# src-d/kmcuda

Hardware: AMD Instinct MI355X
Metric: point-assignments/sec per Lloyd iter (8Mx256@1024) (higher is better)
Workload: dtype f32

## Files before the change

include/kmcuda_amd.h:

```cpp
#ifndef KMCUDA_AMD_H
#define KMCUDA_AMD_H

#include <stddef.h>
#include <stdint.h>

#ifdef __cplusplus
extern "C" {
#endif

typedef struct kmamd_engine kmamd_engine;

int kmamd_engine_create(kmamd_engine **out, int device, uint32_t n_rows, uint32_t features,
                        uint32_t clusters, int metric, int fp16x2, void *hip_stream);
void kmamd_engine_destroy(kmamd_engine *e);
void *kmamd_engine_stream(kmamd_engine *e);
int kmamd_engine_sync(kmamd_engine *e);

int kmamd_lloyd_assign(kmamd_engine *e, const float *samples, const float *centroids,
                       uint32_t *assignments, uint32_t *assignments_prev);
int kmamd_lloyd_assign_exact(kmamd_engine *e, const float *samples, const float *centroids,
                             uint32_t *assignments, uint32_t *assignments_prev);

int kmamd_set_filter(kmamd_engine *e, int mode);

int kmamd_set_half_rows(kmamd_engine *e, const void *rows16);

int kmamd_set_row_cache(kmamd_engine *e, int on);

int kmamd_counters_read(kmamd_engine *e, uint32_t *host_out4);
int kmamd_counters_reset(kmamd_engine *e, int which );
int kmamd_yy_hint_stats(kmamd_engine *e, uint32_t *host_out6);

int kmamd_move_deltas(kmamd_engine *e, const float *samples, const uint32_t *assignments_prev,
                      const uint32_t *assignments, double *delta, int32_t *dcount);
int kmamd_apply_delta(kmamd_engine *e, const double *delta, const int32_t *dcount,
                      float *centroids, uint32_t *ccounts);
size_t kmamd_reduce_len(kmamd_engine *e);
int kmamd_reduce_fill(kmamd_engine *e, const float *samples, const uint32_t *assignments_prev,
                      const uint32_t *assignments, double *buf);
int kmamd_reduce_apply(kmamd_engine *e, const double *buf, float *centroids, uint32_t *ccounts);
int kmamd_reduce_apply_stop(kmamd_engine *e, const double *buf, float *centroids, uint32_t *ccounts,
                            float stop_threshold, uint32_t seq);
int kmamd_stop_report(kmamd_engine *e, uint32_t seq, uint32_t *host_out6);
int kmamd_reduce_apply_prepare(kmamd_engine *e, const double *buf, float *centroids, uint32_t *ccounts,
                               float stop_threshold, uint32_t seq);
int kmamd_stop_clear(kmamd_engine *e);

int kmamd_set_weights(kmamd_engine *e, const float *weights);
int kmamd_centroids_written(kmamd_engine *e);
int kmamd_set_carry(kmamd_engine *e, int on);
int kmamd_carry_stats(kmamd_engine *e, uint64_t *rows_spared, uint32_t *last_list);
int kmamd_carry_pair_stats(kmamd_engine *e, uint64_t *rows_paired);
int kmamd_duo_rows(kmamd_engine *e, uint32_t *rows);
int kmamd_carry_policy_sim(uint32_t n_passes, uint32_t n_rows, float list_max, const uint32_t *list_len, uint32_t lag,
                           uint8_t *out, const uint32_t *changed);
int kmamd_set_update_mode(kmamd_engine *e, int mode);

int kmamd_adjust_exact(kmamd_engine *e, const float *samples, const uint32_t *assignments_prev,
                       const uint32_t *assignments, float *centroids, uint32_t *ccounts);

int kmamd_yy_configure(kmamd_engine *e, uint32_t G, const uint32_t *groups_host);
int kmamd_yy_init(kmamd_engine *e, const float *samples, const float *centroids, const uint32_t *assignments,
                  float *bounds);
int kmamd_yy_drifts(kmamd_engine *e, const float *centroids, float *drifts, float *gdrifts);
int kmamd_yy_filters(kmamd_engine *e, const float *samples, const float *centroids, const float *drifts,
                     const float *gdrifts, uint32_t *assignments, uint32_t *assignments_prev, float *bounds,
                     uint32_t *passed);

int kmamd_afkmc2_draws(kmamd_engine *e, uint64_t seed, uint64_t offset, uint32_t threads, uint32_t n, uint32_t *out);

int kmamd_transpose(kmamd_engine *e, const float *in, uint32_t rows, uint32_t cols, float *out);

int kmamd_filter_kind(kmamd_engine *e, uint32_t *padded_width);

int kmamd_profile_reset(kmamd_engine *e);
int kmamd_profile_read(kmamd_engine *e, double *filter_ms, uint32_t *filter_launches,
                       double *exact_ms, double *update_ms);
int kmamd_profile_read_coarse(kmamd_engine *e, double *coarse_ms);
int kmamd_profile_enable(kmamd_engine *e, int on);

int kmamd_last_run_stats(uint32_t *iterations, double *loop_seconds, double *setup_seconds, uint32_t *shards,
                         uint32_t *rccl_ranks);

int kmamd_kmeans_weighted(int init, const void *init_params, float tolerance, float yinyang_t, int metric,
                          uint32_t samples_size, uint16_t features_size, uint32_t clusters_size, uint32_t seed,
                          uint32_t device, int32_t device_ptrs, int32_t fp16x2, int32_t verbosity, const float *samples,
// ... 30 lines not shown
```

kmcuda_amd/_lib.py:

```python
import ctypes
import os

_HERE = os.path.dirname(os.path.abspath(__file__))
LIB_PATH = os.environ.get("KMCUDA_AMD_LIB") or os.path.join(_HERE, "libKMCUDA.so")

u32, i32, f32 = ctypes.c_uint32, ctypes.c_int32, ctypes.c_float
vp = ctypes.c_void_p

_lib = None

EXPORTS = [
    "kmeans_cuda", "knn_cuda", "kmamd_kmeans_weighted", "kmamd_set_weights",
    "kmamd_engine_create", "kmamd_engine_destroy", "kmamd_engine_stream", "kmamd_engine_sync",
    "kmamd_lloyd_assign", "kmamd_lloyd_assign_exact", "kmamd_set_half_rows", "kmamd_set_row_cache", "kmamd_profile_read_coarse", "kmamd_set_filter", "kmamd_counters_read", "kmamd_counters_reset", "kmamd_yy_hint_stats",
    "kmamd_move_deltas", "kmamd_apply_delta", "kmamd_transpose", "kmamd_afkmc2_draws", "kmamd_reduce_len", "kmamd_reduce_fill",
    "kmamd_reduce_apply", "kmamd_reduce_apply_stop", "kmamd_reduce_apply_prepare", "kmamd_stop_report", "kmamd_stop_clear", "kmamd_centroids_written", "kmamd_set_carry", "kmamd_carry_stats", "kmamd_carry_pair_stats", "kmamd_duo_rows", "kmamd_carry_policy_sim", "kmamd_set_update_mode", "kmamd_last_run_stats", "kmamd_last_run_collective", "kmamd_adjust_exact", "kmamd_yy_configure", "kmamd_yy_init", "kmamd_yy_drifts", "kmamd_yy_filters",
    "kmamd_knn_index_create", "kmamd_knn_index_query", "kmamd_knn_index_destroy",
    "kmamd_knn_index_radius_count", "kmamd_knn_index_radius_fill",
    "kmamd_copy_to_device", "kmamd_profile_reset", "kmamd_profile_read", "kmamd_profile_enable", "kmamd_filter_kind", "kmamd_build_arch",
]


def lib():
    global _lib
    if _lib is not None:
        return _lib
    if not os.path.exists(LIB_PATH):
        raise ImportError(
            "kmcuda_amd: %s is missing -- the HIP library has not been built "
            "(run `make -C kmcuda_amd/csrc`); there is no CPU fallback." % LIB_PATH)
    L = ctypes.CDLL(LIB_PATH, mode=ctypes.RTLD_GLOBAL)
    L.kmeans_cuda.restype = i32
    L.kmeans_cuda.argtypes = [i32, vp, f32, f32, i32, u32, ctypes.c_uint16, u32, u32, u32, i32, i32, i32,
                              vp, vp, vp, vp]
    L.kmamd_kmeans_weighted.restype = i32
    L.kmamd_kmeans_weighted.argtypes = [i32, vp, f32, f32, i32, u32, ctypes.c_uint16, u32, u32, u32, i32, i32, i32,
                                        vp, vp, vp, vp, vp]
    L.kmamd_set_weights.restype = i32
    L.kmamd_set_weights.argtypes = [vp, vp]
    L.knn_cuda.restype = i32
    L.knn_cuda.argtypes = [ctypes.c_uint16, i32, u32, ctypes.c_uint16, u32, u32, i32, i32, i32, vp, vp, vp, vp]
    L.kmamd_engine_create.restype = i32
    L.kmamd_engine_create.argtypes = [ctypes.POINTER(vp), i32, u32, u32, u32, i32, i32, vp]
    L.kmamd_engine_destroy.restype = None
    L.kmamd_engine_destroy.argtypes = [vp]
    L.kmamd_engine_stream.restype = vp
    L.kmamd_engine_stream.argtypes = [vp]
    L.kmamd_engine_sync.restype = i32
    L.kmamd_engine_sync.argtypes = [vp]
# ... 11 lines not shown
    L.kmamd_counters_read.argtypes = [vp, ctypes.POINTER(u32)]
    L.kmamd_counters_reset.restype = i32
    L.kmamd_counters_reset.argtypes = [vp, i32]
    L.kmamd_yy_hint_stats.restype = i32
    L.kmamd_yy_hint_stats.argtypes = [vp, vp]
    L.kmamd_move_deltas.restype = i32
    L.kmamd_move_deltas.argtypes = [vp, vp, vp, vp, vp, vp]
    L.kmamd_apply_delta.restype = i32
    L.kmamd_apply_delta.argtypes = [vp, vp, vp, vp, vp]
    L.kmamd_reduce_len.restype = ctypes.c_size_t
    L.kmamd_reduce_len.argtypes = [vp]
    L.kmamd_reduce_fill.restype = i32
    L.kmamd_reduce_fill.argtypes = [vp, vp, vp, vp, vp]
    L.kmamd_reduce_apply.restype = i32
    L.kmamd_reduce_apply.argtypes = [vp, vp, vp, vp]
    L.kmamd_reduce_apply_stop.restype = i32
    L.kmamd_reduce_apply_stop.argtypes = [vp, vp, vp, vp, f32, u32]
    L.kmamd_reduce_apply_prepare.restype = i32
    L.kmamd_reduce_apply_prepare.argtypes = [vp, vp, vp, vp, f32, u32]
    L.kmamd_stop_report.restype = i32
    L.kmamd_stop_report.argtypes = [vp, u32, ctypes.POINTER(u32)]
    L.kmamd_stop_clear.restype = i32
    L.kmamd_stop_clear.argtypes = [vp]
    L.kmamd_centroids_written.restype = i32
    L.kmamd_centroids_written.argtypes = [vp]
    L.kmamd_set_carry.restype = i32
    L.kmamd_set_carry.argtypes = [vp, i32]
    L.kmamd_carry_stats.restype = i32
    L.kmamd_carry_stats.argtypes = [vp, ctypes.POINTER(ctypes.c_uint64), ctypes.POINTER(ctypes.c_uint32)]
    L.kmamd_carry_pair_stats.restype = i32
    L.kmamd_carry_pair_stats.argtypes = [vp, ctypes.POINTER(ctypes.c_uint64)]
    L.kmamd_duo_rows.restype = i32
    L.kmamd_duo_rows.argtypes = [vp, ctypes.POINTER(ctypes.c_uint32)]
    L.kmamd_carry_policy_sim.restype = i32
    L.kmamd_carry_policy_sim.argtypes = [ctypes.c_uint32, ctypes.c_uint32, ctypes.c_float, ctypes.POINTER(ctypes.c_uint32),
                                         ctypes.c_uint32, ctypes.POINTER(ctypes.c_uint8), ctypes.POINTER(ctypes.c_uint32)]
    L.kmamd_set_update_mode.restype = i32
    L.kmamd_set_update_mode.argtypes = [vp, i32]
    L.kmamd_last_run_stats.restype = i32
    L.kmamd_last_run_stats.argtypes = [ctypes.POINTER(u32), ctypes.POINTER(ctypes.c_double),
                                       ctypes.POINTER(ctypes.c_double), ctypes.POINTER(u32), ctypes.POINTER(u32)]
    L.kmamd_last_run_collective.restype = i32
    L.kmamd_last_run_collective.argtypes = [ctypes.POINTER(ctypes.c_double), ctypes.POINTER(u32)]
    L.kmamd_afkmc2_draws.restype = i32
    L.kmamd_afkmc2_draws.argtypes = [vp, ctypes.c_uint64, ctypes.c_uint64, u32, u32, vp]
    L.kmamd_transpose.restype = i32
    L.kmamd_transpose.argtypes = [vp, vp, u32, u32, vp]
    L.kmamd_adjust_exact.restype = i32
    L.kmamd_adjust_exact.argtypes = [vp, vp, vp, vp, vp, vp]
    L.kmamd_yy_init.restype = i32
    L.kmamd_yy_configure.restype = i32
    L.kmamd_yy_configure.argtypes = [vp, u32, vp]
    L.kmamd_yy_init.argtypes = [vp, vp, vp, vp, vp]
    L.kmamd_yy_drifts.restype = i32
    L.kmamd_yy_drifts.argtypes = [vp, vp, vp, vp]
    L.kmamd_yy_filters.restype = i32
    L.kmamd_yy_filters.argtypes = [vp, vp, vp, vp, vp, vp, vp, vp, vp]
    L.kmamd_profile_reset.restype = i32
    L.kmamd_profile_reset.argtypes = [vp]
    L.kmamd_filter_kind.restype = i32
    L.kmamd_filter_kind.argtypes = [vp, ctypes.POINTER(ctypes.c_uint32)]
    L.kmamd_profile_enable.restype = i32
    L.kmamd_profile_enable.argtypes = [vp, i32]
    L.kmamd_profile_read_coarse.restype = i32
    L.kmamd_profile_read_coarse.argtypes = [vp, ctypes.POINTER(ctypes.c_double)]
    L.kmamd_profile_read.restype = i32
# ... 27 lines not shown
```

kmcuda_amd/csrc/engine.cpp:

```cpp
#include "engine.hpp"

#include <math.h>
#include <stdio.h>
#include <stdlib.h>
#include <string.h>

#include <mutex>
#include <vector>

#include "../../include/kmcuda_amd.h"

namespace kmx {

int g_verbosity = 0;

namespace {
std::mutex g_stream_pool_mutex;
std::vector<std::vector<hipStream_t>> g_stream_pool;
}

hipStream_t pooled_stream_acquire(int device) {
  {
    std::lock_guard<std::mutex> lock(g_stream_pool_mutex);
    if ((size_t)device < g_stream_pool.size() && !g_stream_pool[device].empty()) {
// ... 820 lines not shown
  if (report) KMX_HIP(hipEventRecord(ev_report_[seq & 1u], stream_), kRuntimeError);
  prepared_for_ = centroids;
  return kSuccess;
}

int Engine::carry_stats(unsigned long long *rows_spared, uint32_t *last_list) {
  KMX_HIP(hipSetDevice(device_), kNoSuchDevice);
  unsigned long long v = 0;
  KMX_HIP(hipMemcpyAsync(&v, counters_ + kCarrySkipped, sizeof(v), hipMemcpyDeviceToHost, stream_), kMemoryCopyError);
  KMX_HIP(hipStreamSynchronize(stream_), kRuntimeError);
  if (rows_spared) *rows_spared = v;
  if (last_list) *last_list = host_carry_ ? host_carry_[0] : 0xFFFFFFFFu;
  return kSuccess;
}

int Engine::carry_pair_stats(unsigned long long *rows_paired) {
  KMX_HIP(hipSetDevice(device_), kNoSuchDevice);
  unsigned long long v = 0;
  KMX_HIP(hipMemcpyAsync(&v, counters_ + kCarryPaired, sizeof(v), hipMemcpyDeviceToHost, stream_), kMemoryCopyError);
  KMX_HIP(hipStreamSynchronize(stream_), kRuntimeError);
  if (rows_paired) *rows_paired = v;
  return kSuccess;
}

int Engine::duo_rows(uint32_t *rows) {
  KMX_HIP(hipSetDevice(device_), kNoSuchDevice);
  uint32_t v = 0;
  KMX_HIP(hipMemcpyAsync(&v, counters_ + kDuoCount, sizeof(v), hipMemcpyDeviceToHost, stream_), kMemoryCopyError);
  KMX_HIP(hipStreamSynchronize(stream_), kRuntimeError);
  if (rows) *rows = v;
  return kSuccess;
}

int Engine::set_weights(const float *weights) {
  KMX_HIP(hipSetDevice(device_), kNoSuchDevice);
  weights_ = nullptr;
  weight_total_ = 0.0;
  if (!weights) return kSuccess;
  if (!cweights_) {
    int rc;
    if ((rc = alloc(&cweights_, K_)) || (rc = alloc(&wtail_, (size_t)K_ + 1)) || (rc = alloc(&win_, K_)) ||
        (rc = alloc(&wcheck_, weights_check_doubles())))
      return rc;
  }
  double res[2] = {0.0, 0.0};
  KMX_HIP(launch_weights_check(weights, N_, wcheck_, stream_), kRuntimeError);
  KMX_HIP(hipMemcpyAsync(res, wcheck_, sizeof(res), hipMemcpyDeviceToHost, stream_), kMemoryCopyError);
  KMX_HIP(hipMemsetAsync(cweights_, 0, K_ * sizeof(double), stream_), kRuntimeError);
  KMX_HIP(hipStreamSynchronize(stream_), kRuntimeError);
  if (res[1] != 0.0) return kInvalidArguments;
  weights_ = weights;
  weight_total_ = res[0];
  return kSuccess;
}

int Engine::stop_clear() {
  KMX_HIP(hipSetDevice(device_), kNoSuchDevice);
  carry_valid_ = false;
  KMX_HIP(hipMemsetAsync(counters_ + kStopFlag, 0, sizeof(uint32_t), stream_), kRuntimeError);
  return kSuccess;
}

int Engine::adjust_exact(const float *samples, const uint32_t *prev, const uint32_t *cur, float *centroids,
                         uint32_t *ccounts) {
  KMX_HIP(hipSetDevice(device_), kNoSuchDevice);
  if (strict_h2_) {
// ... 137 lines not shown
  std::vector<uint32_t> reported(n_passes + 1, kmx::CarryPolicy::kNoList);
  std::vector<bool> has_report(n_passes + 1, false);
  bool valid = false;
  for (uint32_t i = 0; i < n_passes; i++) {
    const uint32_t seq = i + 1;
    if (changed && i >= lag) policy.note_changed(changed[i - lag]);
    if (policy.paused()) {
      out[i] = 0;
      valid = false;
      continue;
    }
    if (!valid) {
      out[i] = 1;
      reported[seq] = kmx::CarryPolicy::kNoList;
    } else {
      uint32_t last = kmx::CarryPolicy::kNoList, last_seq = 0;
      for (uint32_t q = seq > lag ? seq - lag : 0; q >= 1; q--)
        if (has_report[q]) { last = reported[q]; last_seq = q; break; }
      out[i] = policy.decide(last, last_seq, seq, n_rows) ? 3 : 2;
      reported[seq] = list_len[i];
    }
    has_report[seq] = true;
    valid = true;
  }
  return kmx::kSuccess;
}
int kmamd_carry_pair_stats(kmamd_engine *e, uint64_t *rows_paired) {
  unsigned long long v = 0;
  const int rc = e->e.carry_pair_stats(&v);
  if (rows_paired) *rows_paired = v;
  return rc;
}
int kmamd_duo_rows(kmamd_engine *e, uint32_t *rows) { return e->e.duo_rows(rows); }
int kmamd_set_update_mode(kmamd_engine *e, int mode) {
  if (mode < 0 || mode > 3) return kmx::kInvalidArguments;
  e->e.ms_.force = mode;
  return kmx::kSuccess;
}
int kmamd_set_filter(kmamd_engine *e, int mode) {
  if (mode < 0 || mode > 1) return kmx::kInvalidArguments;
  e->e.filter_mode_ = mode;
  e->e.prepared_for_ = nullptr;
  return kmx::kSuccess;
}
int kmamd_set_half_rows(kmamd_engine *e, const void *rows16) {
  e->e.half_rows_ = rows16;
  e->e.prepared_for_ = nullptr;
  e->e.row_cache_valid_ = false;
  return kmx::kSuccess;
}
int kmamd_set_row_cache(kmamd_engine *e, int on) {
  e->e.row_cache_on_ = on != 0 && e->e.row_cache_allowed_;
  e->e.row_cache_valid_ = false;
  e->e.prepared_for_ = nullptr;
  if (!e->e.row_cache_on_) e->e.mu_frozen_ = false;
  return kmx::kSuccess;
}
int kmamd_adjust_exact(kmamd_engine *e, const float *samples, const uint32_t *assignments_prev,
                       const uint32_t *assignments, float *centroids, uint32_t *ccounts) {
  return e->e.adjust_exact(samples, assignments_prev, assignments, centroids, ccounts);
}
int kmamd_afkmc2_draws(kmamd_engine *e, uint64_t seed, uint64_t offset, uint32_t threads, uint32_t n, uint32_t *out) {
  if (hipSetDevice(e->e.device_) != hipSuccess) return kmx::kNoSuchDevice;
  return kmx::launch_afk_draws(seed, offset, threads, n, out, e->e.stream_) == hipSuccess ? kmx::kSuccess : kmx::kRuntimeError;
}
int kmamd_transpose(kmamd_engine *e, const float *in, uint32_t rows, uint32_t cols, float *out) {
// ... 55 lines not shown
```

kmcuda_amd/csrc/engine.hpp:

```cpp
#pragma once
#include <hip/hip_runtime.h>
#include <stdint.h>

#include <vector>

#include "kernels.hpp"

namespace kmx {

enum Result {
  kSuccess = 0, kInvalidArguments, kNoSuchDevice, kMemoryAllocationFailure, kRuntimeError, kMemoryCopyError
};

#define KMX_HIP(call, ret)                                                                   \
  do {                                                                                       \
    hipError_t e__ = (call);                                                                 \
    if (e__ != hipSuccess) {                                                                 \
      if (kmx::g_verbosity > 0)                                                              \
        printf("%s:%d -> %s (%s)\n", __FILE__, __LINE__, hipGetErrorString(e__), #call);     \
      return ret;                                                                            \
    }                                                                                        \
  } while (0)

extern int g_verbosity;
// ... 117 lines not shown
  float *und_thr_ = nullptr;
  uint32_t *duo_ = nullptr;
  bool duo_on_ = true;
  bool duo_always_ = false;
  uint32_t coarse_mfma_ = 16;
  int filter_mode_ = 0;
  bool settle_ = true;
  uint32_t wide_dp_ = 0;
  bool wide_ok_ = true;
  bool wide_failed_ = false;
  void *wide_rows16_ = nullptr;
  float *wide_meta_ = nullptr;
  uint32_t *wide_cont_ = nullptr;
  int lloyd_assign_wide(const LloydArgs &a, const float *centroids, bool steady, bool rows_on_side, bool carry_was_valid);
  bool row_cache_allowed_ = true;
  bool row_cache_on_ = false, row_cache_valid_ = false, mu_frozen_ = false;
  void *xcache_ = nullptr;
  float *xmeta_ = nullptr;
  bool carry_on_ = false;
  bool carry_valid_ = false;
  uint32_t carry_preps_ = 0;
  uint32_t carry_seq_ = 0;
  CarryPolicy carry_policy_;
  float *ub_ = nullptr, *lb_ = nullptr, *drift_ = nullptr;
  bool carry_pairs_ = true;
  float *l3_ = nullptr;
  uint32_t *p1_ = nullptr, *p2_ = nullptr;
  uint32_t *carry_list_ = nullptr;
  uint32_t *host_carry_ = nullptr, *host_carry_dev_ = nullptr;
  bool carry_usable() const;
  int carry_stats(unsigned long long *rows_spared, uint32_t *last_list);
  int carry_pair_stats(unsigned long long *rows_paired);
  int duo_rows(uint32_t *rows);
  uint32_t *stats_base_ = nullptr, *stats_ = nullptr, *flagged_ = nullptr, *pairs_ = nullptr, *counters_ = nullptr;
  uint32_t *keys_tmp_ = nullptr, *vals_tmp_ = nullptr, *keys_sorted_ = nullptr, *rows_sorted_ = nullptr,
           *offsets2_ = nullptr, *move_blocks_ = nullptr, *bucket_work_ = nullptr, *bucket_rows_ = nullptr;
  uint32_t bucket_cap_ = 0;
  uint32_t last_undecided_ = 0xFFFFFFFFu;
  MoveState ms_;
  uint32_t *host_move_count_ = nullptr;
  void *sort_temp_ = nullptr;
  size_t sort_temp_bytes_ = 0;
  uint32_t G_ = 0, nslots_ = 0;
  bool yy_exact_ = false;
  bool yy_hint_ = true;
  uint32_t *gfirst_ = nullptr, *gsecond_ = nullptr, *yy_flag_rows_ = nullptr;
  float *yy_hint_buf_ = nullptr;
  void *yy_panelhi_ = nullptr;
  int yy_hint_stats(uint32_t *host6);
  uint32_t *groups_ = nullptr, *cperm_ = nullptr, *gstart_ = nullptr, *pids_ = nullptr, *pmeta_ = nullptr;
  float *pfil_ = nullptr, *pbias_ = nullptr, *xt_ = nullptr;
  float *exact_work_ = nullptr;
  uint32_t *host_counters_ = nullptr;
  uint32_t *host_report_ = nullptr;
  uint32_t *host_report_dev_ = nullptr;
  hipEvent_t ev_report_[2] = {nullptr, nullptr};
  uint32_t *yy_stats_ = nullptr;

  bool profile_ = false;
  double filter_ms_ = 0, exact_ms_ = 0, update_ms_ = 0, coarse_ms_ = 0;
  uint32_t filter_launches_ = 0;
  struct Span { hipEvent_t a, b; int kind; };
  std::vector<Span> spans_;
  std::vector<size_t> open_spans_;
  void span_begin(int kind);
  void span_end();
// ... 15 lines not shown
```

kmcuda_amd/csrc/lloyd_duo.hip:

```cpp
#include <hip/hip_runtime.h>

#include "filter_common.hpp"
#include "kernels.hpp"

namespace kmx {

typedef float f32x4 __attribute__((ext_vector_type(4)));

__device__ __forceinline__ float row16_sum(float v) {
  v += __int_as_float(__builtin_amdgcn_update_dpp(0, __float_as_int(v), 0xB1, 0xF, 0xF, true));
  v += __int_as_float(__builtin_amdgcn_update_dpp(0, __float_as_int(v), 0x4E, 0xF, 0xF, true));
  v += __int_as_float(__builtin_amdgcn_update_dpp(0, __float_as_int(v), 0x141, 0xF, 0xF, true));
  v += __int_as_float(__builtin_amdgcn_update_dpp(0, __float_as_int(v), 0x140, 0xF, 0xF, true));
  return v;
}

constexpr uint32_t kDuoPend = 64;

template <int NI, bool FAST, bool BOUNDS = false>
__global__ __launch_bounds__(256, NI >= 4 ? 2 : 4) void lloyd_duo_kernel(
    const float *__restrict__ samples, uint32_t D, uint32_t DP, uint32_t K, const float *__restrict__ cfil,
    const float *__restrict__ bias, const float *__restrict__ mu, const uint32_t *__restrict__ stats, float eps,
    float tie_slack, const uint4 *__restrict__ duo, uint32_t *__restrict__ assignments,
    uint32_t *__restrict__ assignments_prev, uint32_t *__restrict__ flagged, uint32_t *__restrict__ pairs,
    uint32_t *__restrict__ counters, CarryArgs cy) {
  if (counters[kStopFlag] != 0u) return;
  constexpr int SLOTS = NI >= 8 ? 1 : 2;
  const uint32_t total = counters[kDuoCount];
  const uint32_t lane = threadIdx.x & 63, wave = threadIdx.x >> 6, g = lane >> 4, l = lane & 15;
  const float cmaxc = sqrtf(__uint_as_float(stats[0])) * 1.000001f;
  const float bmaxc = __uint_as_float(stats[1]);
  const float cmaxo = sqrtf(__uint_as_float(stats[2])) * 1.000001f;
  const float u = 5.9604645e-8f;
  const bool angular = tie_slack > 0.f;
  float mreg[NI][4];
#pragma unroll
  for (int i = 0; i < NI; i++) {
    const uint32_t f = 64u * i + 4u * l;
#pragma unroll
    for (int e = 0; e < 4; e++) mreg[i][e] = f + e < DP ? mu[f + e] : 0.f;
  }
  __shared__ uint32_t pbuf[4][kDuoPend * 3], fbuf[4][kDuoPend], blk_n[4][3], blk_base[2];
  uint32_t *mypairs = pbuf[wave], *myflags = fbuf[wave];
  uint32_t np = 0, nf = 0, nchg = 0;
  auto flush = [&](uint32_t *list_counter, uint32_t *list, const uint32_t *buf, uint32_t words_each, uint32_t &n) {
    if (n == 0) return;
    uint32_t base = 0;
    if (lane == 0) base = atomicAdd(list_counter, n);
    base = __shfl(base, 0);
    for (uint32_t i = lane; i < n * words_each; i += 64) list[words_each * (size_t)base + i] = buf[i];
    n = 0;
  };
    const uint32_t per_iter = 4u * SLOTS;
  uint4 rec_next[SLOTS];
  auto request = [&](uint32_t base) {
#pragma unroll
    for (int k = 0; k < SLOTS; k++) {
      const uint32_t p = base + 4u * k + g;
      rec_next[k] = p < total ? duo[p] : make_uint4(0u, 0u, 0u, 0u);
    }
  };
  request((blockIdx.x * 4u + wave) * per_iter);
  for (uint32_t base = (blockIdx.x * 4u + wave) * per_iter; base < total; base += gridDim.x * 4u * per_iter) {
    uint4 rec[SLOTS];
    bool live[SLOTS];
    f32x4 xv[SLOTS][NI], c1v[SLOTS][NI], c2v[SLOTS][NI];
    uint32_t old_asg[SLOTS];
    float bias_a[SLOTS], bias_b[SLOTS];
#pragma unroll
    for (int k = 0; k < SLOTS; k++) {
      live[k] = base + 4u * k + g < total;
      rec[k] = rec_next[k];
    }
    request(base + gridDim.x * 4u * per_iter);
#pragma unroll
    for (int k = 0; k < SLOTS; k++) {
      old_asg[k] = assignments[rec[k].x];
      bias_a[k] = bias[rec[k].y];
      bias_b[k] = bias[rec[k].z];
    }
#pragma unroll
    for (int k = 0; k < SLOTS; k++) {
      const float *xr = samples + (size_t)rec[k].x * D;
      const float *r1 = cfil + (size_t)rec[k].y * DP, *r2 = cfil + (size_t)rec[k].z * DP;
#pragma unroll
      for (int i = 0; i < NI; i++) {
        const uint32_t f = 64u * i + 4u * l;
        f32x4 x = {0.f, 0.f, 0.f, 0.f}, a = x, b = x;
        if (f < DP) {
          if (FAST) {
            x = __builtin_nontemporal_load(reinterpret_cast<const f32x4 *>(xr + f));
          } else {
            x.x = f + 0 < D ? xr[f + 0] : 0.f; x.y = f + 1 < D ? xr[f + 1] : 0.f;
            x.z = f + 2 < D ? xr[f + 2] : 0.f; x.w = f + 3 < D ? xr[f + 3] : 0.f;
          }
          a = *reinterpret_cast<const f32x4 *>(r1 + f);
          b = *reinterpret_cast<const f32x4 *>(r2 + f);
        }
        xv[k][i] = x; c1v[k][i] = a; c2v[k][i] = b;
      }
    }
#pragma unroll
    for (int k = 0; k < SLOTS; k++) {
      float xn2 = 0.f, xo2 = 0.f, p1 = 0.f, p2 = 0.f, xdm = 0.f, xab = 0.f, nan0 = 0.f;
#pragma unroll
      for (int i = 0; i < NI; i++) {
        const float x4[4] = {xv[k][i].x, xv[k][i].y, xv[k][i].z, xv[k][i].w};
        const float a4[4] = {c1v[k][i].x, c1v[k][i].y, c1v[k][i].z, c1v[k][i].w};
        const float b4[4] = {c2v[k][i].x, c2v[k][i].y, c2v[k][i].z, c2v[k][i].w};
#pragma unroll
        for (int e = 0; e < 4; e++) {
          const float xc = x4[e] - mreg[i][e];
          xn2 = fmaf(xc, xc, xn2);
          xo2 = fmaf(x4[e], x4[e], xo2);
          p1 = fmaf(xc, a4[e], p1);
          p2 = fmaf(xc, b4[e], p2);
          if (angular) {
            xdm = fmaf(x4[e], mreg[i][e], xdm);
            xab = fmaf(fabsf(x4[e]), fabsf(mreg[i][e]), xab);
          }
        }
        if (i == 0 && l == 0 && x4[0] != x4[0]) nan0 = 1.f;
      }
      xn2 = row16_sum(xn2); xo2 = row16_sum(xo2); p1 = row16_sum(p1); p2 = row16_sum(p2); nan0 = row16_sum(nan0);
      if (angular) { xdm = row16_sum(xdm); xab = row16_sum(xab); }
      const uint32_t s = rec[k].x, ca = rec[k].y, cb = rec[k].z;
      const float va = p1 + bias_a[k], vb = p2 + bias_b[k];
      float v1 = va, v2 = -INFINITY;
      const float v3 = -INFINITY;
      uint32_t i1 = ca, i2 = 0xFFFFFFFFu;
      if (!(va > -INFINITY)) { v1 = -INFINITY; i1 = 0xFFFFFFFFu; }
      {
        const bool g1 = vb > v1, g2 = vb > v2;
        i2 = g1 ? i1 : (g2 ? cb : i2);
        v2 = g1 ? v1 : (g2 ? vb : v2);
        i1 = g1 ? cb : i1;
        v1 = g1 ? vb : v1;
      }
      const bool insane = nan0 > 0.f;
      const float xn = sqrtf(xn2) * 1.0001f, xo = sqrtf(xo2) * 1.0001f;
      const float e_mfma = 2.0f * eps * (xn * cmaxc + bmaxc);
      const float e_ref = u * (12.0f * xo * cmaxo + 4.0f * cmaxo * cmaxo);
      const float thr = 2.0f * (e_mfma + e_ref) * 1.001f + tie_slack;
      const bool in_range = (xn < 6.0e4f) && (cmaxc < 6.0e4f) && i1 < K;
      const ClampLimits lim = clamp_limits(angular, xdm, dot_error((int)DP, xab), 0.5f * thr);
      const bool certain = insane || (in_range && ((v1 - v2) > thr) && (v2 < lim.hi) && (v1 > lim.lo));
      const bool two = !certain && in_range && ((v1 - v3) > thr) && (v3 < lim.hi) && (v1 > lim.lo) && i2 < K;
      const bool mine = live[k] && l == 0;
      const bool pair_now = mine && two, flag_now = mine && !certain && !two;
      if (mine && certain) {
        const uint32_t nearest = insane ? K : i1;
        assignments_prev[s] = old_asg[k];
        if (old_asg[k] != nearest) {
          assignments[s] = nearest;
          nchg++;
        }
      }
      if constexpr (BOUNDS) {
        if (mine) {
          const float rest = __uint_as_float(rec[k].w);
          const bool ok = !insane && in_range && (certain || two);
          const float e = e_mfma * 1.001f;
          const float dcmax = sqrtf(__uint_as_float(stats[5])) * 1.000001f, dxw = 4.8829e-4f * xn;
          const float e_c = 2.0f * eps * (xn * cmaxc + bmaxc) + (xn * dcmax + dxw * cmaxc + dxw * dcmax) * 1.001f +
                            6e-8f * sqrtf((float)DP) * (xn + cmaxc) + 2.0e-6f * (1.001f * xn * cmaxc + bmaxc);
          const float w = fmaxf(rest + e_c * 1.001f, v3 + e);
          if (cy.angular) {
            float pairg = 0.f;
            if (ok && i2 < K) pairg = fminf(fminf((v2 - e) - w, lim.hi - w), v2 - lim.lo) * 0.999999f;
            if (!(pairg > 0.f)) pairg = 0.f;
            cy.ub[s] = -INFINITY;
            cy.l3[s] = pairg;
            if (pairg > 0.f) { cy.p1[s] = i1; cy.p2[s] = i2; }
          } else {
            float ubv = INFINITY, l3v = 0.f;
            if (ok) {
              const float geo = 2.4e-7f * (xn + cmaxc);
              const float d2l = xn2 * (1.0f - 2.0f * eps) - 2.0f * w;
              float low = d2l > 0.f ? fmaxf(sqrtf(d2l) * 0.999999f - geo, 0.f) : 0.f;
              if (!(low == low)) low = 0.f;
              ubv = sqrtf(fmaxf(xn2 * (1.0f + 2.0f * eps) - 2.0f * (v2 - e), 0.f)) * 1.000001f + geo;
              if (!(ubv == ubv)) ubv = INFINITY;
              if (i2 < K) l3v = low;
            }
            cy.ub[s] = ubv;
            cy.lb[s] = 0.f;
            cy.l3[s] = l3v;
            if (l3v > 0.f) { cy.p1[s] = i1; cy.p2[s] = i2; }
          }
        }
      }
      const unsigned long long pm = __ballot(pair_now), fm = __ballot(flag_now);
      if (pm) {
        if (np + 4 > kDuoPend) flush(&counters[3], pairs, mypairs, 3, np);
        if (pair_now) {
          const uint32_t at = np + (uint32_t)__popcll(pm & ((1ull << lane) - 1ull));
          mypairs[3 * at + 0] = s; mypairs[3 * at + 1] = i1; mypairs[3 * at + 2] = i2;
        }
        np += (uint32_t)__popcll(pm);
      }
      if (fm) {
        if (nf + 4 > kDuoPend) flush(&counters[1], flagged, myflags, 1, nf);
        if (flag_now) myflags[nf + (uint32_t)__popcll(fm & ((1ull << lane) - 1ull))] = s;
        nf += (uint32_t)__popcll(fm);
      }
    }
  }
#pragma unroll
  for (int off = 32; off > 0; off >>= 1) nchg += __shfl_xor(nchg, off);
  if (lane == 0) { blk_n[wave][0] = np; blk_n[wave][1] = nf; blk_n[wave][2] = nchg; }
  __syncthreads();
  if (threadIdx.x == 0) {
    uint32_t tp = 0, tf = 0, tc = 0;
    for (int w = 0; w < 4; w++) { tp += blk_n[w][0]; tf += blk_n[w][1]; tc += blk_n[w][2]; }
    blk_base[0] = tp ? atomicAdd(&counters[3], tp) : 0u;
    blk_base[1] = tf ? atomicAdd(&counters[1], tf) : 0u;
    if (tc) atomicAdd(&counters[0], tc);
  }
  __syncthreads();
  uint32_t bp = blk_base[0], bf = blk_base[1];
  for (uint32_t w = 0; w < wave; w++) { bp += blk_n[w][0]; bf += blk_n[w][1]; }
  for (uint32_t i = lane; i < np * 3; i += 64) pairs[3 * (size_t)bp + i] = mypairs[i];
  for (uint32_t i = lane; i < nf; i += 64) flagged[bf + i] = myflags[i];
}

template <int NI>
static hipError_t launch_duo_ni(const LloydArgs &a, const uint32_t *duo, hipStream_t st, const CarryArgs *cy) {
  const bool fast = a.D == a.DP && (((uintptr_t)a.samples) & 15u) == 0 && a.DP % 4 == 0;
  const uint32_t want = (a.N + 31u) / 32u, full = NI >= 4 ? 512u : 1024u;
  const dim3 grid(want < full ? (want ? want : 1u) : full);
#define KMX_DUO_LAUNCH(F, B, CY)                                                                                      \
  hipLaunchKernelGGL((lloyd_duo_kernel<NI, F, B>), grid, dim3(256), 0, st, a.samples, a.D, a.DP, a.K, a.cfil, a.bias,    \
                     a.mu, a.stats, a.eps, a.tie_slack, reinterpret_cast<const uint4 *>(duo), a.assignments,          \
                     a.assignments_prev, a.flagged, a.pairs, a.counters, CY)
  if (cy && cy->l3) {
    if (fast) KMX_DUO_LAUNCH(true, true, *cy); else KMX_DUO_LAUNCH(false, true, *cy);
  } else {
    if (fast) KMX_DUO_LAUNCH(true, false, CarryArgs()); else KMX_DUO_LAUNCH(false, false, CarryArgs());
  }
#undef KMX_DUO_LAUNCH
  return hipGetLastError();
}

hipError_t launch_lloyd_duo(const LloydArgs &a, const uint32_t *duo, hipStream_t st, const CarryArgs *cy) {
  if (a.N == 0) return hipSuccess;
  switch (a.DP) {
    case 16: case 32: case 64: return launch_duo_ni<1>(a, duo, st, cy);
    case 128: return launch_duo_ni<2>(a, duo, st, cy);
    case 256: return launch_duo_ni<4>(a, duo, st, cy);
    case 512: return launch_duo_ni<8>(a, duo, st, cy);
    default: return hipErrorInvalidValue;
  }
}

hipError_t preload_lloyd_duo_code() {
  hipFuncAttributes at;
  return hipFuncGetAttributes(&at, reinterpret_cast<const void *>(&lloyd_duo_kernel<4, true>));
}

}
```

kmcuda_amd/engine.py:

```python
import ctypes

import torch

from . import _lib

L2, COS = 0, 1
_METRICS = {"L2": L2, "l2": L2, "euclidean": L2, "cos": COS, "cosine": COS, "angular": COS}


def metric_id(metric):
    if isinstance(metric, int):
        return metric
    return _METRICS[metric]


class Engine:

    def __init__(self, n_rows, features, clusters, metric="L2", device=0, use_torch_stream=True):
        self.lib = _lib.lib()
        self.n_rows, self.features, self.clusters = int(n_rows), int(features), int(clusters)
        self.metric = metric_id(metric)
        self.device = torch.device("cuda", device)
        stream = None
        if use_torch_stream:
# ... 27 lines not shown
        fn = self.lib.kmamd_lloyd_assign_exact if exact else self.lib.kmamd_lloyd_assign
        _lib.check(fn(self.h, self._p(samples), self._p(centroids), self._p(assignments), self._p(assignments_prev)),
                   "kmamd_lloyd_assign")

    def set_filter(self, mode):
        _lib.check(self.lib.kmamd_set_filter(self.h, {"f16": 0, "f32": 1}[mode]), "kmamd_set_filter")

    def set_half_rows(self, rows16):
        self._half_rows = rows16
        _lib.check(self.lib.kmamd_set_half_rows(self.h, self._p(rows16) if rows16 is not None else None),
                   "kmamd_set_half_rows")

    def set_row_cache(self, on=True):
        _lib.check(self.lib.kmamd_set_row_cache(self.h, 1 if on else 0), "kmamd_set_row_cache")

    def set_carry(self, on=True):
        _lib.check(self.lib.kmamd_set_carry(self.h, 1 if on else 0), "kmamd_set_carry")

    def carry_stats(self):
        spared, last = ctypes.c_uint64(0), ctypes.c_uint32(0)
        _lib.check(self.lib.kmamd_carry_stats(self.h, ctypes.byref(spared), ctypes.byref(last)), "kmamd_carry_stats")
        return int(spared.value), int(last.value)

    def carry_pair_stats(self):
        paired = ctypes.c_uint64(0)
        _lib.check(self.lib.kmamd_carry_pair_stats(self.h, ctypes.byref(paired)), "kmamd_carry_pair_stats")
        return int(paired.value)

    def duo_rows(self):
        rows = ctypes.c_uint32(0)
        _lib.check(self.lib.kmamd_duo_rows(self.h, ctypes.byref(rows)), "kmamd_duo_rows")
        return int(rows.value)

    def counters(self):
        out = (ctypes.c_uint32 * 4)()
        _lib.check(self.lib.kmamd_counters_read(self.h, out), "kmamd_counters_read")
        return list(out)

    def reset_counters(self, which=-1):
        _lib.check(self.lib.kmamd_counters_reset(self.h, which), "kmamd_counters_reset")

    def move_deltas(self, samples, prev, cur, delta, dcount):
        _lib.check(self.lib.kmamd_move_deltas(self.h, self._p(samples), self._p(prev), self._p(cur), self._p(delta),
                                              self._p(dcount)), "kmamd_move_deltas")

    def apply_delta(self, delta, dcount, centroids, ccounts):
        _lib.check(self.lib.kmamd_apply_delta(self.h, self._p(delta), self._p(dcount), self._p(centroids),
                                              self._p(ccounts)), "kmamd_apply_delta")

    def set_weights(self, weights):
        if weights is not None and (weights.dtype != torch.float32 or weights.dim() != 1
                                    or weights.shape[0] != self.n_rows or not weights.is_contiguous()):
            raise ValueError("weights must be a contiguous 1-D float32 tensor of n_rows elements")
        rc = self.lib.kmamd_set_weights(self.h, self._p(weights) if weights is not None else None)
        if rc == 1:
            raise ValueError("sample weights must be finite and > 0")
        _lib.check(rc, "kmamd_set_weights")
        self._weights = weights

    def adjust_exact(self, samples, prev, cur, centroids, ccounts):
        _lib.check(self.lib.kmamd_adjust_exact(self.h, self._p(samples), self._p(prev), self._p(cur),
                                               self._p(centroids), self._p(ccounts)), "kmamd_adjust_exact")

    def reduce_len(self):
        return int(self.lib.kmamd_reduce_len(self.h))

# ... 78 lines not shown
```

Baseline: 2.201 billion.

## Software-pipeline duo kernel row and centroid fetches with ring of prefetched groups

New measurement: 2.205 billion, median of 6. About the same (+0.2%).

```diff
diff --git a/include/kmcuda_amd.h b/include/kmcuda_amd.h
--- a/include/kmcuda_amd.h
+++ b/include/kmcuda_amd.h
@@ -52,6 +52,7 @@
 int kmamd_carry_stats(kmamd_engine *e, uint64_t *rows_spared, uint32_t *last_list);
 int kmamd_carry_pair_stats(kmamd_engine *e, uint64_t *rows_paired);
 int kmamd_duo_rows(kmamd_engine *e, uint32_t *rows);
+int kmamd_undecided_rows(kmamd_engine *e, uint32_t *rows);
 int kmamd_carry_policy_sim(uint32_t n_passes, uint32_t n_rows, float list_max, const uint32_t *list_len, uint32_t lag,
                            uint8_t *out, const uint32_t *changed);
 int kmamd_set_update_mode(kmamd_engine *e, int mode);
diff --git a/kmcuda_amd/_lib.py b/kmcuda_amd/_lib.py
--- a/kmcuda_amd/_lib.py
+++ b/kmcuda_amd/_lib.py
@@ -14,7 +14,7 @@
     "kmamd_engine_create", "kmamd_engine_destroy", "kmamd_engine_stream", "kmamd_engine_sync",
     "kmamd_lloyd_assign", "kmamd_lloyd_assign_exact", "kmamd_set_half_rows", "kmamd_set_row_cache", "kmamd_profile_read_coarse", "kmamd_set_filter", "kmamd_counters_read", "kmamd_counters_reset", "kmamd_yy_hint_stats",
     "kmamd_move_deltas", "kmamd_apply_delta", "kmamd_transpose", "kmamd_afkmc2_draws", "kmamd_reduce_len", "kmamd_reduce_fill",
-    "kmamd_reduce_apply", "kmamd_reduce_apply_stop", "kmamd_reduce_apply_prepare", "kmamd_stop_report", "kmamd_stop_clear", "kmamd_centroids_written", "kmamd_set_carry", "kmamd_carry_stats", "kmamd_carry_pair_stats", "kmamd_duo_rows", "kmamd_carry_policy_sim", "kmamd_set_update_mode", "kmamd_last_run_stats", "kmamd_last_run_collective", "kmamd_adjust_exact", "kmamd_yy_configure", "kmamd_yy_init", "kmamd_yy_drifts", "kmamd_yy_filters",
+    "kmamd_reduce_apply", "kmamd_reduce_apply_stop", "kmamd_reduce_apply_prepare", "kmamd_stop_report", "kmamd_stop_clear", "kmamd_centroids_written", "kmamd_set_carry", "kmamd_carry_stats", "kmamd_carry_pair_stats", "kmamd_duo_rows", "kmamd_undecided_rows", "kmamd_carry_policy_sim", "kmamd_set_update_mode", "kmamd_last_run_stats", "kmamd_last_run_collective", "kmamd_adjust_exact", "kmamd_yy_configure", "kmamd_yy_init", "kmamd_yy_drifts", "kmamd_yy_filters",
     "kmamd_knn_index_create", "kmamd_knn_index_query", "kmamd_knn_index_destroy",
     "kmamd_knn_index_radius_count", "kmamd_knn_index_radius_fill",
     "kmamd_copy_to_device", "kmamd_profile_reset", "kmamd_profile_read", "kmamd_profile_enable", "kmamd_filter_kind", "kmamd_build_arch",
@@ -92,6 +92,8 @@
     L.kmamd_carry_pair_stats.argtypes = [vp, ctypes.POINTER(ctypes.c_uint64)]
     L.kmamd_duo_rows.restype = i32
     L.kmamd_duo_rows.argtypes = [vp, ctypes.POINTER(ctypes.c_uint32)]
+    L.kmamd_undecided_rows.restype = i32
+    L.kmamd_undecided_rows.argtypes = [vp, ctypes.POINTER(ctypes.c_uint32)]
     L.kmamd_carry_policy_sim.restype = i32
     L.kmamd_carry_policy_sim.argtypes = [ctypes.c_uint32, ctypes.c_uint32, ctypes.c_float, ctypes.POINTER(ctypes.c_uint32),
                                          ctypes.c_uint32, ctypes.POINTER(ctypes.c_uint8), ctypes.POINTER(ctypes.c_uint32)]
diff --git a/kmcuda_amd/csrc/engine.cpp b/kmcuda_amd/csrc/engine.cpp
--- a/kmcuda_amd/csrc/engine.cpp
+++ b/kmcuda_amd/csrc/engine.cpp
@@ -876,6 +876,15 @@
   return kSuccess;
 }
 
+int Engine::undecided_rows(uint32_t *rows) {
+  KMX_HIP(hipSetDevice(device_), kNoSuchDevice);
+  uint32_t v = 0;
+  KMX_HIP(hipMemcpyAsync(&v, counters_ + 4, sizeof(v), hipMemcpyDeviceToHost, stream_), kMemoryCopyError);
+  KMX_HIP(hipStreamSynchronize(stream_), kRuntimeError);
+  if (rows) *rows = v;
+  return kSuccess;
+}
+
 int Engine::set_weights(const float *weights) {
   KMX_HIP(hipSetDevice(device_), kNoSuchDevice);
   weights_ = nullptr;
@@ -1079,6 +1088,7 @@
   return rc;
 }
 int kmamd_duo_rows(kmamd_engine *e, uint32_t *rows) { return e->e.duo_rows(rows); }
+int kmamd_undecided_rows(kmamd_engine *e, uint32_t *rows) { return e->e.undecided_rows(rows); }
 int kmamd_set_update_mode(kmamd_engine *e, int mode) {
   if (mode < 0 || mode > 3) return kmx::kInvalidArguments;
   e->e.ms_.force = mode;
diff --git a/kmcuda_amd/csrc/engine.hpp b/kmcuda_amd/csrc/engine.hpp
--- a/kmcuda_amd/csrc/engine.hpp
+++ b/kmcuda_amd/csrc/engine.hpp
@@ -173,6 +173,7 @@
   int carry_stats(unsigned long long *rows_spared, uint32_t *last_list);
   int carry_pair_stats(unsigned long long *rows_paired);
   int duo_rows(uint32_t *rows);
+  int undecided_rows(uint32_t *rows);
   uint32_t *stats_base_ = nullptr, *stats_ = nullptr, *flagged_ = nullptr, *pairs_ = nullptr, *counters_ = nullptr;
   uint32_t *keys_tmp_ = nullptr, *vals_tmp_ = nullptr, *keys_sorted_ = nullptr, *rows_sorted_ = nullptr,
            *offsets2_ = nullptr, *move_blocks_ = nullptr, *bucket_work_ = nullptr, *bucket_rows_ = nullptr;
diff --git a/kmcuda_amd/csrc/lloyd_duo.hip b/kmcuda_amd/csrc/lloyd_duo.hip
--- a/kmcuda_amd/csrc/lloyd_duo.hip
+++ b/kmcuda_amd/csrc/lloyd_duo.hip
@@ -18,29 +18,27 @@
 constexpr uint32_t kDuoPend = 64;
 
 template <int NI, bool FAST, bool BOUNDS = false>
-__global__ __launch_bounds__(256, NI >= 4 ? 2 : 4) void lloyd_duo_kernel(
+__global__ __launch_bounds__(256, 2) void lloyd_duo_kernel(
     const float *__restrict__ samples, uint32_t D, uint32_t DP, uint32_t K, const float *__restrict__ cfil,
     const float *__restrict__ bias, const float *__restrict__ mu, const uint32_t *__restrict__ stats, float eps,
     float tie_slack, const uint4 *__restrict__ duo, uint32_t *__restrict__ assignments,
     uint32_t *__restrict__ assignments_prev, uint32_t *__restrict__ flagged, uint32_t *__restrict__ pairs,
     uint32_t *__restrict__ counters, CarryArgs cy) {
   if (counters[kStopFlag] != 0u) return;
-  constexpr int SLOTS = NI >= 8 ? 1 : 2;
+  constexpr int CA = NI >= 8 || (NI == 4 && !FAST) ? 0 : 1, CSETS = CA + 1;
+  constexpr int AHEAD = NI >= 8 ? 0 : NI == 4 ? (FAST ? 1 : 2) : 3, SETS = AHEAD + 1;
+  constexpr int UNROLL = SETS % CSETS == 0 ? SETS : SETS * CSETS;
   const uint32_t total = counters[kDuoCount];
-  const uint32_t lane = threadIdx.x & 63, wave = threadIdx.x >> 6, g = lane >> 4, l = lane & 15;
+  const uint32_t lane = threadIdx.x & 63, wave = __builtin_amdgcn_readfirstlane(threadIdx.x >> 6), g = lane >> 4, l = lane & 15;
   const float cmaxc = sqrtf(__uint_as_float(stats[0])) * 1.000001f;
   const float bmaxc = __uint_as_float(stats[1]);
   const float cmaxo = sqrtf(__uint_as_float(stats[2])) * 1.000001f;
   const float u = 5.9604645e-8f;
   const bool angular = tie_slack > 0.f;
-  float mreg[NI][4];
-#pragma unroll
-  for (int i = 0; i < NI; i++) {
-    const uint32_t f = 64u * i + 4u * l;
-#pragma unroll
-    for (int e = 0; e < 4; e++) mreg[i][e] = f + e < DP ? mu[f + e] : 0.f;
-  }
+  __shared__ f32x4 mu_lds[NI * 16];
   __shared__ uint32_t pbuf[4][kDuoPend * 3], fbuf[4][kDuoPend], blk_n[4][3], blk_base[2];
+  for (uint32_t f = threadIdx.x; f < 64u * NI; f += 256u) reinterpret_cast<float *>(mu_lds)[f] = f < DP ? mu[f] : 0.f;
+  __syncthreads();
   uint32_t *mypairs = pbuf[wave], *myflags = fbuf[wave];
   uint32_t np = 0, nf = 0, nchg = 0;
   auto flush = [&](uint32_t *list_counter, uint32_t *list, const uint32_t *buf, uint32_t words_each, uint32_t &n) {
@@ -51,81 +49,97 @@
     for (uint32_t i = lane; i < n * words_each; i += 64) list[words_each * (size_t)base + i] = buf[i];
     n = 0;
   };
-    const uint32_t per_iter = 4u * SLOTS;
-  uint4 rec_next[SLOTS];
+  const uint32_t stride = gridDim.x * 16u;
+  struct Group {
+    uint4 rec;
+    f32x4 xv[NI];
+    uint32_t old_asg;
+    float bias_a, bias_b;
+  };
   auto request = [&](uint32_t base) {
-#pragma unroll
-    for (int k = 0; k < SLOTS; k++) {
-      const uint32_t p = base + 4u * k + g;
-      rec_next[k] = p < total ? duo[p] : make_uint4(0u, 0u, 0u, 0u);
-    }
-  };
-  request((blockIdx.x * 4u + wave) * per_iter);
-  for (uint32_t base = (blockIdx.x * 4u + wave) * per_iter; base < total; base += gridDim.x * 4u * per_iter) {
-    uint4 rec[SLOTS];
-    bool live[SLOTS];
-    f32x4 xv[SLOTS][NI], c1v[SLOTS][NI], c2v[SLOTS][NI];
-    uint32_t old_asg[SLOTS];
-    float bias_a[SLOTS], bias_b[SLOTS];
-#pragma unroll
-    for (int k = 0; k < SLOTS; k++) {
-      live[k] = base + 4u * k + g < total;
-      rec[k] = rec_next[k];
-    }
-    request(base + gridDim.x * 4u * per_iter);
-#pragma unroll
-    for (int k = 0; k < SLOTS; k++) {
-      old_asg[k] = assignments[rec[k].x];
-      bias_a[k] = bias[rec[k].y];
-      bias_b[k] = bias[rec[k].z];
-    }
-#pragma unroll
-    for (int k = 0; k < SLOTS; k++) {
-      const float *xr = samples + (size_t)rec[k].x * D;
-      const float *r1 = cfil + (size_t)rec[k].y * DP, *r2 = cfil + (size_t)rec[k].z * DP;
+    const uint32_t p = base + g;
+    const bool in = p < total;
+    const uint4 r = duo[in ? p : 0u];
+    return make_uint4(in ? r.x : 0u, in ? r.y : 0u, in ? r.z : 0u, in ? r.w : 0u);
+  };
+  auto has = [&](uint32_t f) { return NI > 1 || f < DP; };
+  const f32x4 zero = {0.f, 0.f, 0.f, 0.f};
+  auto fetch_rows = [&](Group &t) {
+    t.old_asg = assignments[t.rec.x];
+    t.bias_a = bias[t.rec.y];
+    t.bias_b = bias[t.rec.z];
+    const float *xr = samples + (size_t)t.rec.x * D;
+#pragma unroll
+    for (int i = 0; i < NI; i++) {
+      const uint32_t f = 64u * i + 4u * l;
+      f32x4 x;
+      if (FAST) {
+        x = __builtin_nontemporal_load(reinterpret_cast<const f32x4 *>(xr + (has(f) ? f : 0u)));
+        x = has(f) ? x : zero;
+      } else {
+        const float *pad = mu + (has(f) ? f : 0u);
+        x.x = *(f + 0 < D ? xr + f + 0 : pad + 0); x.y = *(f + 1 < D ? xr + f + 1 : pad + 1);
+        x.z = *(f + 2 < D ? xr + f + 2 : pad + 2); x.w = *(f + 3 < D ? xr + f + 3 : pad + 3);
+        x = has(f) ? x : zero;
+        __builtin_amdgcn_sched_barrier(0);
+      }
+      t.xv[i] = x;
+    }
+  };
+  struct Pair {
+    f32x4 c1v[NI], c2v[NI];
+  };
+  auto fetch_pair = [&](const uint4 &rec, Pair &t) {
+    const float *r1 = cfil + (size_t)rec.y * DP, *r2 = cfil + (size_t)rec.z * DP;
+#pragma unroll
+    for (int i = 0; i < NI; i++) {
+      const uint32_t f = 64u * i + 4u * l, fo = has(f) ? f : 0u;
+      const f32x4 a = *reinterpret_cast<const f32x4 *>(r1 + fo);
+      const f32x4 b = *reinterpret_cast<const f32x4 *>(r2 + fo);
+      t.c1v[i] = has(f) ? a : zero; t.c2v[i] = has(f) ? b : zero;
+    }
+  };
+  uint4 rec_ahead;
+  auto step = [&](uint32_t base, Group &cur, Group &fill, const Pair &ccur, const Group &cnext, Pair &cfill) {
+    fill.rec = rec_ahead;
+    rec_ahead = request(base + (uint32_t)(AHEAD + 1) * stride);
+    const uint4 rec = cur.rec;
+    const bool live = base + g < total;
+    fetch_pair(cnext.rec, cfill);
+    __builtin_amdgcn_sched_barrier(0);
+    fetch_rows(fill);
+    __builtin_amdgcn_sched_barrier(0);
+    const f32x4 (&c1v)[NI] = ccur.c1v, (&c2v)[NI] = ccur.c2v;
+    const f32x4 (&xv)[NI] = cur.xv;
+    const uint32_t old_asg = cur.old_asg;
+    const float bias_a = cur.bias_a, bias_b = cur.bias_b;
+    {
+      float xn2 = 0.f, xo2 = 0.f, p1 = 0.f, p2 = 0.f, xdm = 0.f, xab = 0.f, nan0 = 0.f;
 #pragma unroll
       for (int i = 0; i < NI; i++) {
-        const uint32_t f = 64u * i + 4u * l;
-        f32x4 x = {0.f, 0.f, 0.f, 0.f}, a = x, b = x;
-        if (f < DP) {
-          if (FAST) {
-            x = __builtin_nontemporal_load(reinterpret_cast<const f32x4 *>(xr + f));
-          } else {
-            x.x = f + 0 < D ? xr[f + 0] : 0.f; x.y = f + 1 < D ? xr[f + 1] : 0.f;
-            x.z = f + 2 < D ? xr[f + 2] : 0.f; x.w = f + 3 < D ? xr[f + 3] : 0.f;
-          }
-          a = *reinterpret_cast<const f32x4 *>(r1 + f);
-          b = *reinterpret_cast<const f32x4 *>(r2 + f);
-        }
-        xv[k][i] = x; c1v[k][i] = a; c2v[k][i] = b;
-      }
-    }
-#pragma unroll
-    for (int k = 0; k < SLOTS; k++) {
-      float xn2 = 0.f, xo2 = 0.f, p1 = 0.f, p2 = 0.f, xdm = 0.f, xab = 0.f, nan0 = 0.f;
-#pragma unroll
-      for (int i = 0; i < NI; i++) {
-        const float x4[4] = {xv[k][i].x, xv[k][i].y, xv[k][i].z, xv[k][i].w};
-        const float a4[4] = {c1v[k][i].x, c1v[k][i].y, c1v[k][i].z, c1v[k][i].w};
-        const float b4[4] = {c2v[k][i].x, c2v[k][i].y, c2v[k][i].z, c2v[k][i].w};
+        const float x4[4] = {xv[i].x, xv[i].y, xv[i].z, xv[i].w};
+        const float a4[4] = {c1v[i].x, c1v[i].y, c1v[i].z, c1v[i].w};
+        const float b4[4] = {c2v[i].x, c2v[i].y, c2v[i].z, c2v[i].w};
+        const f32x4 mv = mu_lds[16 * i + l];
+        const float m4[4] = {mv.x, mv.y, mv.z, mv.w};
 #pragma unroll
         for (int e = 0; e < 4; e++) {
-          const float xc = x4[e] - mreg[i][e];
+          const float xc = x4[e] - m4[e];
           xn2 = fmaf(xc, xc, xn2);
           xo2 = fmaf(x4[e], x4[e], xo2);
           p1 = fmaf(xc, a4[e], p1);
           p2 = fmaf(xc, b4[e], p2);
           if (angular) {
-            xdm = fmaf(x4[e], mreg[i][e], xdm);
-            xab = fmaf(fabsf(x4[e]), fabsf(mreg[i][e]), xab);
+            xdm = fmaf(x4[e], m4[e], xdm);
+            xab = fmaf(fabsf(x4[e]), fabsf(m4[e]), xab);
           }
         }
         if (i == 0 && l == 0 && x4[0] != x4[0]) nan0 = 1.f;
       }
       xn2 = row16_sum(xn2); xo2 = row16_sum(xo2); p1 = row16_sum(p1); p2 = row16_sum(p2); nan0 = row16_sum(nan0);
       if (angular) { xdm = row16_sum(xdm); xab = row16_sum(xab); }
-      const uint32_t s = rec[k].x, ca = rec[k].y, cb = rec[k].z;
-      const float va = p1 + bias_a[k], vb = p2 + bias_b[k];
+      const uint32_t s = rec.x, ca = rec.y, cb = rec.z;
+      const float va = p1 + bias_a, vb = p2 + bias_b;
       float v1 = va, v2 = -INFINITY;
       const float v3 = -INFINITY;
       uint32_t i1 = ca, i2 = 0xFFFFFFFFu;
@@ -146,19 +160,19 @@
       const ClampLimits lim = clamp_limits(angular, xdm, dot_error((int)DP, xab), 0.5f * thr);
       const bool certain = insane || (in_range && ((v1 - v2) > thr) && (v2 < lim.hi) && (v1 > lim.lo));
       const bool two = !certain && in_range && ((v1 - v3) > thr) && (v3 < lim.hi) && (v1 > lim.lo) && i2 < K;
-      const bool mine = live[k] && l == 0;
+      const bool mine = live && l == 0;
       const bool pair_now = mine && two, flag_now = mine && !certain && !two;
       if (mine && certain) {
         const uint32_t nearest = insane ? K : i1;
-        assignments_prev[s] = old_asg[k];
-        if (old_asg[k] != nearest) {
+        assignments_prev[s] = old_asg;
+        if (old_asg != nearest) {
           assignments[s] = nearest;
           nchg++;
         }
       }
       if constexpr (BOUNDS) {
         if (mine) {
-          const float rest = __uint_as_float(rec[k].w);
+          const float rest = __uint_as_float(rec.w);
           const bool ok = !insane && in_range && (certain || two);
           const float e = e_mfma * 1.001f;
           const float dcmax = sqrtf(__uint_as_float(stats[5])) * 1.000001f, dxw = 4.8829e-4f * xn;
@@ -205,7 +219,29 @@
         nf += (uint32_t)__popcll(fm);
       }
     }
-  }
+  };
+  static_assert(CA <= AHEAD, "a group's record is there before its centroid rows are requested");
+  Group st[SETS];
+  Pair cs[CSETS];
+  uint32_t base = (blockIdx.x * 4u + wave) * 4u;
+#pragma unroll
+  for (int r = 0; r < AHEAD; r++) st[r].rec = request(base + (uint32_t)r * stride);
+  rec_ahead = request(base + (uint32_t)AHEAD * stride);
+  if (base < total) {
+#pragma unroll
+    for (int r = 0; r < CA; r++) fetch_pair(st[r].rec, cs[r]);
+#pragma unroll
+    for (int r = 0; r < AHEAD; r++) fetch_rows(st[r]);
+  }
+  while (base < total) {
+#pragma unroll
+    for (int r = 0; r < UNROLL; r++) {
+      step(base, st[r % SETS], st[(r + AHEAD) % SETS], cs[r % CSETS], st[(r + CA) % SETS], cs[(r + CA) % CSETS]);
+      base += stride;
+      if (r + 1 < UNROLL && base >= total) goto list_done;
+    }
+  }
+list_done:
 #pragma unroll
   for (int off = 32; off > 0; off >>= 1) nchg += __shfl_xor(nchg, off);
   if (lane == 0) { blk_n[wave][0] = np; blk_n[wave][1] = nf; blk_n[wave][2] = nchg; }
@@ -227,7 +263,7 @@
 template <int NI>
 static hipError_t launch_duo_ni(const LloydArgs &a, const uint32_t *duo, hipStream_t st, const CarryArgs *cy) {
   const bool fast = a.D == a.DP && (((uintptr_t)a.samples) & 15u) == 0 && a.DP % 4 == 0;
-  const uint32_t want = (a.N + 31u) / 32u, full = NI >= 4 ? 512u : 1024u;
+  const uint32_t want = (a.N + 15u) / 16u, full = 384u;
   const dim3 grid(want < full ? (want ? want : 1u) : full);
 #define KMX_DUO_LAUNCH(F, B, CY)                                                                                      \
   hipLaunchKernelGGL((lloyd_duo_kernel<NI, F, B>), grid, dim3(256), 0, st, a.samples, a.D, a.DP, a.K, a.cfil, a.bias,    \
diff --git a/kmcuda_amd/engine.py b/kmcuda_amd/engine.py
--- a/kmcuda_amd/engine.py
+++ b/kmcuda_amd/engine.py
@@ -83,6 +83,11 @@
         _lib.check(self.lib.kmamd_duo_rows(self.h, ctypes.byref(rows)), "kmamd_duo_rows")
         return int(rows.value)
 
+    def undecided_rows(self):
+        rows = ctypes.c_uint32(0)
+        _lib.check(self.lib.kmamd_undecided_rows(self.h, ctypes.byref(rows)), "kmamd_undecided_rows")
+        return int(rows.value)
+
     def counters(self):
         out = (ctypes.c_uint32 * 4)()
         _lib.check(self.lib.kmamd_counters_read(self.h, out), "kmamd_counters_read")
```
